# ecpoppenheimer/TensorFlowRayTrace

Measured on AMD Instinct MI355X. Metric: ray-surface intersection tests/sec (fwd+bwd), higher is better.
Workload: dtype f32 ray state, f32 filter + f64 decisions

## Files before the change

tensorflowraytrace_amd/csrc/tfrt_trace3d.hip:

```cpp
#include <vector>

#include <type_traits>
#include "tfrt_common.h"
#include "goal_finish.h"
#include "wave_schedule.h"

namespace tfrt {

constexpr int TILE = 512;
constexpr int KC = 24;

constexpr int ERR_CAPACITY = 1;


__global__ __launch_bounds__(BLOCK) void k_center(const double* __restrict__ fverts, int M,
                                                  double* __restrict__ c0, int32_t* nrays0, int n,
                                                  int32_t* tail8, unsigned int* scan_ticket) {
  if (nrays0 != nullptr) {
    if (threadIdx.x == 0) *nrays0 = n;
    if (threadIdx.x < 8) tail8[threadIdx.x] = 0;
    if (threadIdx.x == 0 && scan_ticket != nullptr) *scan_ticket = 0u;
  }
  __shared__ double red[WAVES][3];
  __shared__ double ctr[3];
// ... 2552 lines not shown
    } else {
      double* gp = g_fverts + 9 * (int64_t)tri;
#pragma unroll
      for (int c = 0; c < 9; ++c)
        if (gP[c] != 0.0) unsafeAtomicAdd(gp + c, gP[c]);
    }
  }
  wave_fence();
  for (int k0 = 0; k0 < cells; k0 += 64) {
    const int k = k0 + lane;
    double v = k < cells ? wacc[k] : 0.0;
    v += dpp_f64<0xB1>(v);
    if (copies >= 4) v += dpp_f64<0x4E>(v);
    if (copies >= 8) v += dpp_f64<0x141>(v);
    if ((lane & (copies - 1)) == 0 && k < cells && v != 0.0) {
      const int term = k / copies;
      unsafeAtomicAdd(g_fverts + 9 * (int64_t)wface[term / 9] + (term % 9), v);
    }
  }
  wave_fence();
}

template <typename T, int BW>
__global__ __launch_bounds__(64 * BW) void k_backward3d(
    const T* __restrict__ rays_in, int64_t stride_in, const int32_t* __restrict__ n_ptr,
    const int32_t* __restrict__ ray_id_in, const int32_t* __restrict__ rec_tri,
    const double* __restrict__ rec_t, const uint8_t* __restrict__ rec_cls,
    const int32_t* __restrict__ rec_slot, const int32_t* __restrict__ pass_counts,
    tfrt_scene3d sc, double L, double dead_len,
    const typename SweepStore<T>::type* __restrict__ g_child, int64_t child_stride,
    const double* __restrict__ g_fin, int64_t cap_fin, const double* __restrict__ g_act,
    int64_t cap_act, const double* __restrict__ g_stp, int64_t cap_stp,
    const double* __restrict__ g_dead, int64_t cap_dead,
    typename SweepStore<T>::type* __restrict__ g_out, double* __restrict__ g_src_out,
    int64_t out_stride, double* __restrict__ g_fverts,
    typename SweepStore<T>::type* __restrict__ stash_g, int32_t* __restrict__ stash_face,
    int wave_sums) {
  const int n = *n_ptr;
  const int q0 = blockIdx.x * (64 * BW) + threadIdx.x;
  const int i = q0;
  if (wave_sums) {
    if ((q0 & ~63) >= n) return;
    __shared__ double wacc[BW][WSUM_CELLS];
    __shared__ int32_t wface[BW][WSUM_SLOTS];
    const int wave = threadIdx.x >> 6;
    double gP[9];
    int tri = -1;
    if (i < n)
      tri = backward_ray<T>(i, rays_in, stride_in, ray_id_in, rec_tri, rec_t, rec_cls, rec_slot,
                            pass_counts, sc, L, dead_len, g_child, child_stride, g_fin, cap_fin,
                            g_act, cap_act, g_stp, cap_stp, g_dead, cap_dead, g_out, g_src_out,
                            out_stride, gP);
    wave_face_sums(tri, gP, wacc[wave], wface[wave], g_fverts);
    return;
  }
  if (i >= n) return;
  double gP[9];
  const int tri = backward_ray<T>(i, rays_in, stride_in, ray_id_in, rec_tri, rec_t, rec_cls,
                                  rec_slot, pass_counts, sc, L, dead_len, g_child, child_stride,
                                  g_fin, cap_fin, g_act, cap_act, g_stp, cap_stp, g_dead, cap_dead,
                                  g_out, g_src_out, out_stride, gP);
  if (stash_face != nullptr) {
    stash_face[i] = tri;
    if (tri >= 0) {
      using S = typename SweepStore<T>::type;
      S* o = stash_g + 9 * (int64_t)i;
#pragma unroll
      for (int c = 0; c < 9; ++c) o[c] = static_cast<S>(gP[c]);
    }
    return;
  }
  if (tri >= 0) {
    double* gp = g_fverts + 9 * (int64_t)tri;
#pragma unroll
    for (int c = 0; c < 9; ++c) {
      if (gP[c] != 0.0) unsafeAtomicAdd(gp + c, gP[c]);
    }
  }
}

constexpr int FACE_WINDOW = 2048;

template <typename S>
__global__ __launch_bounds__(1024) void k_face_accumulate(
    const int32_t* __restrict__ nrays, int passes, int64_t pass_stride,
    const int32_t* __restrict__ stash_face, const S* __restrict__ stash_g, int chunk, int M,
    double* __restrict__ g_fverts) {
  __shared__ double acc[FACE_WINDOW * 9];
  const int lo = blockIdx.x * chunk;
  if (lo >= nrays[0]) return;
  const int w0 = blockIdx.y * FACE_WINDOW;
  const int w1 = min(M, w0 + FACE_WINDOW);
  for (int k = threadIdx.x; k < FACE_WINDOW * 9; k += 1024) acc[k] = 0.0;
  __syncthreads();
  for (int p = 0; p < passes; ++p) {
    const int hi = min(nrays[p], lo + chunk);
    const int32_t* __restrict__ face = stash_face + (int64_t)p * pass_stride;
    const S* __restrict__ terms = stash_g + 9 * (int64_t)p * pass_stride;
    constexpr int U = 4;
    for (int base = lo + threadIdx.x; base < hi; base += 1024 * U) {
      int t[U];
#pragma unroll
      for (int u = 0; u < U; ++u) {
        const int i = base + u * 1024;
        t[u] = i < hi ? face[i] : -1;
      }
      double g[U][9];
#pragma unroll
      for (int u = 0; u < U; ++u) {
        if (t[u] >= w0 && t[u] < w1) {
          const S* src = terms + 9 * (int64_t)(base + u * 1024);
#pragma unroll
          for (int c = 0; c < 9; ++c) g[u][c] = static_cast<double>(src[c]);
        }
      }
#pragma unroll
      for (int u = 0; u < U; ++u) {
        if (t[u] >= w0 && t[u] < w1) {
          double* a = acc + 9 * (t[u] - w0);
#pragma unroll
          for (int c = 0; c < 9; ++c)
            if (g[u][c] != 0.0) unsafeAtomicAdd(a + c, g[u][c]);
        }
      }
    }
  }
  __syncthreads();
  for (int k = threadIdx.x; k < (w1 - w0) * 9; k += 1024) {
    const double v = acc[k];
    if (v != 0.0) unsafeAtomicAdd(g_fverts + 9 * (int64_t)w0 + k, v);
  }
}

constexpr int FIXED_BITS = 40;

template <typename S>
__global__ __launch_bounds__(BLOCK) void k_stash_absmax(const int32_t* __restrict__ n_ptr,
                                                        const int32_t* __restrict__ stash_face,
                                                        const S* __restrict__ stash_g,
                                                        unsigned long long* __restrict__ maxbits) {
  const int n = *n_ptr;
  const int i = blockIdx.x * BLOCK + threadIdx.x;
  double m = 0.0;
  if (i < n && stash_face[i] >= 0) {
    const S* g = stash_g + 9 * (int64_t)i;
#pragma unroll
    for (int c = 0; c < 9; ++c) {
      const double a = fabs(static_cast<double>(g[c]));
      if (a > m && a < INFINITY) m = a;
    }
  }
#pragma unroll
  for (int d = 32; d > 0; d >>= 1) m = fmax(m, __shfl_xor(m, d, 64));
  if (lane_id() == 0 && m > 0.0) atomicMax(maxbits, (unsigned long long)__double_as_longlong(m));
}

__device__ __forceinline__ double fixed_scale(unsigned long long maxbits) {
  if (maxbits == 0ull) return 0.0;
  int e;
  (void)frexp(__longlong_as_double((long long)maxbits), &e);
  int shift = FIXED_BITS - e;
  if (shift > 1000) shift = 1000;
  return ldexp(1.0, shift);
}

template <typename S>
__global__ __launch_bounds__(BLOCK) void k_face_accumulate_fixed(
    const int32_t* __restrict__ n_ptr, const int32_t* __restrict__ stash_face,
    const S* __restrict__ stash_g, const unsigned long long* __restrict__ maxbits,
    unsigned long long* __restrict__ acc, uint8_t* __restrict__ flag) {
  const int n = *n_ptr;
  const int i = blockIdx.x * BLOCK + threadIdx.x;
  if (i >= n) return;
  const int f = stash_face[i];
  if (f < 0) return;
  const double scale = fixed_scale(*maxbits);
  const S* g = stash_g + 9 * (int64_t)i;
#pragma unroll
  for (int c = 0; c < 9; ++c) {
    const double x = static_cast<double>(g[c]);
    if (!(fabs(x) < INFINITY)) {
      flag[9 * (int64_t)f + c] = 1;
    } else {
      const long long q = llrint(x * scale);
      if (q != 0) atomicAdd(acc + 9 * (int64_t)f + c, (unsigned long long)q);
    }
  }
}

__global__ __launch_bounds__(BLOCK) void k_fixed_finish(int64_t m9,
                                                        const unsigned long long* __restrict__ max_this,
                                                        unsigned long long* __restrict__ max_next,
                                                        unsigned long long* __restrict__ acc,
                                                        uint8_t* __restrict__ flag,
                                                        double* __restrict__ g_fverts) {
  const int64_t i = (int64_t)blockIdx.x * BLOCK + threadIdx.x;
  const double scale = fixed_scale(*max_this);
  if (i < m9) {
    const long long q = (long long)acc[i];
    if (flag[i] != 0) {
      g_fverts[i] = __builtin_nan("");
    } else if (q != 0) {
      g_fverts[i] += (double)q / scale;
    }
    acc[i] = 0ull;
    flag[i] = 0;
  }
  if (i == 0) *max_next = 0ull;
}

template <typename T, bool GN = true>
__device__ __forceinline__ int backward_core(
    int i, int tape, int slot, const T* __restrict__ rays_in, int64_t stride_in,
    const int32_t* __restrict__ ray_id_in, const int32_t* __restrict__ rec_tri,
    const double* __restrict__ rec_t, const int32_t* __restrict__ pass_counts,
    const tfrt_scene3d& sc, double L, double dead_len, bool child_pass, const double child[6],
    const double* seed_fin,
    const double* __restrict__ g_fin, int64_t cap_fin, const double* __restrict__ g_act,
    int64_t cap_act, const double* __restrict__ g_stp, int64_t cap_stp,
    const double* __restrict__ g_dead, int64_t cap_dead, double gs[3], double ge[3],
    double gP[9], int tri_known = -2, const double* __restrict__ feta = nullptr,
    bool slot_global = false) {
  int face_out = -1;
  const int cls = tape & 3;
  double s[3], e[3];
  load_ray3(rays_in, stride_in, i, s, e);
  for (int k = 0; k < 3; ++k) gs[k] = ge[k] = 0.0;
  double P[9], t_rec = 0.0, n_in = 1.0, n_out = 1.0;
  int tri = tri_known;
  auto load_face = [&](bool with_indices) {
    const double* fp = sc.face_verts + 9 * (int64_t)tri;
#pragma unroll
    for (int q = 0; q < 9; ++q) P[q] = fp[q];
    t_rec = rec_t[i];
    if (with_indices) {
      if (feta != nullptr) {
        n_in = feta[4 * (int64_t)tri + 2];
        n_out = feta[4 * (int64_t)tri + 3];
      } else {
        face_indices(sc, tri, ray_id_in ? ray_id_in[i] : i, &n_in, &n_out);
      }
    }
  };
  const bool early = tri_known >= 0 && cls != CLS_DEAD;
  if (early) load_face(child_pass && cls == CLS_ACTIVE);

  if (cls == CLS_DEAD) {
    if (g_dead != nullptr) {
      double a[3] = {0, 0, 0}, b[3] = {0, 0, 0};
      add6(g_dead, cap_dead, slot, a, b);
      const double dl = (dead_len != 0.0) ? dead_len : 1.0;
      for (int k = 0; k < 3; ++k) {
        gs[k] = a[k] + (1.0 - dl) * b[k];
        ge[k] = dl * b[k];
      }
    }
  } else {
    double g_s[3] = {0, 0, 0}, g_h[3] = {0, 0, 0}, g_ce[3] = {0, 0, 0};
    bool has_child = false;
    if (cls == CLS_FINISHED) {
      if (seed_fin != nullptr) {
        for (int k = 0; k < 3; ++k) {
          g_s[k] += seed_fin[k];
          g_h[k] += seed_fin[3 + k];
        }
      } else {
        add6(g_fin, cap_fin, slot, g_s, g_h);
      }
    } else if (cls == CLS_STOPPED) {
      add6(g_stp, cap_stp, slot, g_s, g_h);
    } else {
      if (g_act != nullptr)
        add6(g_act, cap_act, (slot_global ? 0 : (int64_t)pass_counts[4 + CLS_ACTIVE]) + slot, g_s, g_h);
      if (child_pass) {
        has_child = true;
        for (int k = 0; k < 3; ++k) {
          g_h[k] += child[k];
          g_ce[k] += child[3 + k];
        }
      }
    }
    bool nz = has_child;
    for (int k = 0; k < 3; ++k) nz = nz || g_s[k] != 0.0 || g_h[k] != 0.0;
    if (nz) {
      if (!early) {
        if (tri_known < -1) tri = rec_tri[i];
        load_face(has_child);
      }
      double gn[2];
      const bool want_n = GN && has_child && sc.grad_n_in != nullptr && sc.n_table == nullptr;
      const int branch = ((tape & TAPE_INTERNAL) ? 1 : 0) | ((tape & TAPE_REFLECT) ? 2 : 0);
      adjoint3d(s, e, P, t_rec, has_child, n_in, n_out, L, g_s, g_h, g_ce, gs, ge, gP, gn, branch,
                want_n);
      if (want_n) {
        if (gn[0] != 0.0) unsafeAtomicAdd(sc.grad_n_in + tri, gn[0]);
        if (gn[1] != 0.0) unsafeAtomicAdd(sc.grad_n_out + tri, gn[1]);
      }
      if (sc.face_grad_mask == nullptr || sc.face_grad_mask[tri] != 0) face_out = tri;
    }
  }
  return face_out;
}

template <typename T>
__device__ __forceinline__ int backward_ray(
    int i, const T* __restrict__ rays_in, int64_t stride_in, const int32_t* __restrict__ ray_id_in,
    const int32_t* __restrict__ rec_tri, const double* __restrict__ rec_t,
    const uint8_t* __restrict__ rec_cls, const int32_t* __restrict__ rec_slot,
    const int32_t* __restrict__ pass_counts, const tfrt_scene3d& sc, double L, double dead_len,
    const typename SweepStore<T>::type* __restrict__ g_child, int64_t child_stride,
    const double* __restrict__ g_fin, int64_t cap_fin, const double* __restrict__ g_act,
    int64_t cap_act, const double* __restrict__ g_stp, int64_t cap_stp,
    const double* __restrict__ g_dead, int64_t cap_dead,
    typename SweepStore<T>::type* __restrict__ g_out, double* __restrict__ g_src_out,
    int64_t out_stride, double gP[9]) {
  const int tape = rec_cls[i];
  const int slot = rec_slot[i];
  double child[6] = {0, 0, 0, 0, 0, 0};
  const bool child_pass = g_child != nullptr;
  if (child_pass && (tape & 3) == CLS_ACTIVE) {
    for (int k = 0; k < 6; ++k) child[k] = static_cast<double>(g_child[k * child_stride + slot]);
  }
  double gs[3], ge[3];
  const int face_out = backward_core<T>(i, tape, slot, rays_in, stride_in, ray_id_in, rec_tri,
                                        rec_t, pass_counts, sc, L, dead_len, child_pass, child,
                                        nullptr, g_fin, cap_fin, g_act, cap_act, g_stp, cap_stp, g_dead,
                                        cap_dead, gs, ge, gP);
  if (g_out != nullptr) {
    using G = typename SweepStore<T>::type;
    for (int k = 0; k < 3; ++k) {
      g_out[k * out_stride + i] = static_cast<G>(gs[k]);
      g_out[(3 + k) * out_stride + i] = static_cast<G>(ge[k]);
    }
  } else if (g_src_out != nullptr) {
    for (int k = 0; k < 3; ++k) {
      g_src_out[k * out_stride + i] = gs[k];
      g_src_out[(3 + k) * out_stride + i] = ge[k];
    }
  }
  return face_out;
}

constexpr int CHAIN_MAXP = 8;

template <typename T>
struct ChainArgs {
  const T* src;
  int64_t src_stride;
  const T* rays_ws;
  const int32_t* nrays;
  const int32_t* rayid;
  const int32_t* rec_tri;
  const int32_t* rec_slot;
  const double* rec_t;
  const uint8_t* rec_cls;
  const int32_t* counts;
  int64_t n;
  int32_t P;
  double L, dead_len;
  const double *g_fin, *g_act, *g_stp, *g_dead;
  int64_t cap_fin, cap_act, cap_stp, cap_dead;
  double* g_src;
  int64_t N;
  double* g_fverts;
  const T* fin_rays;
  int64_t fin_cap;
  GoalFields gf;
  const double* goal;
  int64_t goal_stride, goal_ray_stride;
  double* partial;
  int32_t* partial_cnt;
  const double* feta;
  int32_t inplace;
  int32_t chain_in_lds;
};

#ifndef TFRT_CHAIN_WAVES
#define TFRT_CHAIN_WAVES 4
#endif
template <typename T, int BW, bool GOAL, bool GN>
__global__ __launch_bounds__(64 * BW)
__attribute__((amdgpu_waves_per_eu(TFRT_CHAIN_WAVES, TFRT_CHAIN_WAVES))) void k_backward_chain(
    ChainArgs<T> a, tfrt_scene3d sc) {
#pragma clang fp contract(off)
  const int n0 = a.nrays[0];
  const int i0 = blockIdx.x * (64 * BW) + threadIdx.x;
  if ((i0 & ~63) >= n0) {
    if (GOAL && (threadIdx.x & 63) == 0) {
      a.partial[i0 >> 6] = 0.0;
      if (a.partial_cnt != nullptr) a.partial_cnt[2 * (i0 >> 6)] = a.partial_cnt[2 * (i0 >> 6) + 1] = 0;
    }
    return;
  }
  __shared__ double wacc[BW][WSUM_CELLS];
  __shared__ int32_t wface[BW][WSUM_SLOTS];
  extern __shared__ int4 chain_lds[];
  const int lane = threadIdx.x & 63, wave = threadIdx.x >> 6;
  const int P = a.P;
  int4* chain = chain_lds + (size_t)wave * P * 64;
  int last = -1;
  if (i0 < n0) {
    int j = i0;
    for (int p = 0; p < P; ++p) {
      const size_t at = (size_t)p * a.n + j;
      const int tape = a.rec_cls[at], tri = a.rec_tri[at];
      const int slot = a.inplace >= 2 ? j : a.rec_slot[at];
      if (a.chain_in_lds) chain[p * 64 + lane] = make_int4(j, tape, slot, tri);
      last = p;
      if ((tape & 3) != CLS_ACTIVE || p == P - 1) break;
      if (!a.inplace) j = slot;
    }
  }
  int top = last;
#pragma unroll
  for (int d = 32; d > 0; d >>= 1) top = max(top, __shfl_xor(top, d, 64));
  double child[6] = {0, 0, 0, 0, 0, 0};
  double err = 0.0;
  int n_fin = 0, n_entered = 0;
  for (int p = top; p >= 0; --p) {
    double gP[9];
    int tri = -1;
    bool fin_here = false;
    if (p <= last) {
      int4 rec;
      if (a.chain_in_lds) {
        rec = chain[p * 64 + lane];
      } else {
        const size_t at = (size_t)p * a.n + i0;
        rec = make_int4(i0, a.rec_cls[at], a.inplace >= 2 ? i0 : a.rec_slot[at], a.rec_tri[at]);
      }
      const int j = rec.x, tape = rec.y, slot = rec.z;
      const size_t off = (size_t)p * a.n;
      const T* rin = p == 0 ? a.src : a.rays_ws + (size_t)(p - 1) * 6 * a.n;
      const int64_t sin = p == 0 ? a.src_stride : a.n;
      const int32_t* idin = (p == 0 || a.inplace) ? nullptr : a.rayid + (size_t)(p - 1) * a.n;
      double seed[6] = {0, 0, 0, 0, 0, 0};
      if (GOAL && p == last && (tape & 3) == CLS_FINISHED) {
        fin_here = true;
        double fin_row[6] = {0, 0, 0, 0, 0, 0};
        if (a.inplace) {
          double s0[3], e0[3], h0[3];
          load_ray3(rin, sin, j, s0, e0);
          hit_point(s0, e0, a.rec_t[off + j], h0);
#pragma unroll
          for (int k = 0; k < 3; ++k) {
            fin_row[k] = s0[k];
            fin_row[3 + k] = static_cast<double>(static_cast<T>(h0[k]));
          }
        }
        for (int c = 0; c < a.gf.n; ++c) {
          const int row = a.gf.row[c];
          double out_c = 0.0;
          if (a.inplace) {
#pragma unroll
            for (int k = 0; k < 6; ++k)
              if (k == row) out_c = fin_row[k];
          } else {
            out_c = ldd(a.fin_rays, (int64_t)row * a.fin_cap + slot);
          }
          const double r = out_c -
                           a.goal[(int64_t)c * a.goal_stride + (int64_t)i0 * a.goal_ray_stride];
          const double g = 2.0 * r;
#pragma unroll
          for (int q = 0; q < 6; ++q)
            if (q == row) seed[q] = g;
          err += r * r;
        }
      }
      double gs[3], ge[3];
      tri = backward_core<T, GN>(j, tape, slot, rin, sin, idin, a.rec_tri + off, a.rec_t + off,
                                 a.counts + (size_t)p * TFRT_COUNTS_PER_PASS, sc, a.L, a.dead_len,
                                 p < P - 1, child, GOAL ? seed : nullptr, a.g_fin, a.cap_fin, a.g_act,
                             a.cap_act, a.g_stp, a.cap_stp, a.g_dead, a.cap_dead, gs, ge, gP,
                             rec.w, a.feta, a.inplace != 0);
      for (int k = 0; k < 3; ++k) {
        child[k] = gs[k];
        child[3 + k] = ge[k];
      }
    }
    if (GOAL) {
      n_fin += __popcll(__ballot(fin_here));
      n_entered += __popcll(__ballot(p <= last));
    }
    wave_face_sums(tri, gP, wacc[wave], wface[wave], a.g_fverts);
  }
  if (a.g_src != nullptr && i0 < n0) {
    for (int k = 0; k < 6; ++k) a.g_src[k * a.N + i0] = child[k];
  }
  if (GOAL) {
#pragma unroll
    for (int d = 32; d > 0; d >>= 1) err += __shfl_xor(err, d, 64);
    if (lane == 0) {
      a.partial[i0 >> 6] = err;
      if (a.partial_cnt != nullptr) {
        a.partial_cnt[2 * (i0 >> 6)] = n_fin;
        a.partial_cnt[2 * (i0 >> 6) + 1] = n_entered;
      }
    }
  }
}

template <typename T>
struct ChainGoalArgs {
  const T* src;
  int64_t src_stride;
  const T* rays_ws;
  const int32_t* nrays;
  const int32_t* rec_tri;
  const double* rec_t;
  const uint8_t* rec_cls;
  int64_t n;
  int32_t P;
  double L;
  double* g_src;
  int64_t N;
  double* g_fverts;
  GoalFields gf;
  const double* goal;
  int64_t goal_stride, goal_ray_stride;
  double* partial;
  int32_t* partial_cnt;
  const double* feta;
  const double* face_verts;
  const uint8_t* face_grad_mask;
  const int32_t* sched;
  int32_t ngroups;
};

template <typename T>
__global__ __launch_bounds__(64)
__attribute__((amdgpu_waves_per_eu(TFRT_CHAIN_WAVES, TFRT_CHAIN_WAVES))) void k_backward_chain_goal_inplace(
    ChainGoalArgs<T> a) {
#pragma clang fp contract(off)
  const int n0 = a.nrays[0];
  int wave = blockIdx.x;
  if (a.sched != nullptr) {
    wave = __builtin_amdgcn_readfirstlane(a.sched[blockIdx.x]);
    if ((unsigned)wave >= (unsigned)a.ngroups) return;
  }
  const int i0 = wave * 64 + threadIdx.x;
  const int lane = threadIdx.x;
  if ((i0 & ~63) >= n0) {
    if (lane == 0) {
      a.partial[i0 >> 6] = 0.0;
      if (a.partial_cnt != nullptr) a.partial_cnt[2 * (i0 >> 6)] = a.partial_cnt[2 * (i0 >> 6) + 1] = 0;
    }
    return;
  }
  __builtin_assume(a.feta != nullptr);
  __shared__ double wacc[WSUM_CELLS];
  __shared__ int32_t wface[WSUM_SLOTS];
  extern __shared__ int2 chain_goal_lds[];
  int2* chain = chain_goal_lds;
  const int P = a.P;
  tfrt_scene3d sc = {};
  sc.face_verts = a.face_verts;
  sc.face_grad_mask = a.face_grad_mask;
  int last = -1;
  if (i0 < n0) {
    for (int p = 0; p < P; ++p) {
      const size_t at = (size_t)p * a.n + i0;
      const int tape = a.rec_cls[at], tri = a.rec_tri[at];
      chain[p * 64 + lane] = make_int2(tape, tri);
      last = p;
      if ((tape & 3) != CLS_ACTIVE) break;
    }
  }
  int top = last;
#pragma unroll
  for (int d = 32; d > 0; d >>= 1) top = max(top, __shfl_xor(top, d, 64));
  top = __builtin_amdgcn_readfirstlane(top);
  double child[6] = {0, 0, 0, 0, 0, 0};
  double err = 0.0;
  int n_fin = 0, n_entered = 0;
  for (int p = top; p >= 0; --p) {
    double gP[9];
    int tri = -1;
    bool fin_here = false;
    if (p <= last) {
      const int2 rec = chain[p * 64 + lane];
      const int tape = rec.x;
      const size_t off = (size_t)p * a.n;
      const T* rin = p == 0 ? a.src : a.rays_ws + (size_t)(p - 1) * 6 * a.n;
      const int64_t sin = p == 0 ? a.src_stride : a.n;
      double seed[6] = {0, 0, 0, 0, 0, 0};
      if (p == last && (tape & 3) == CLS_FINISHED) {
        fin_here = true;
        double fin_row[6], s0[3], e0[3], h0[3];
        load_ray3(rin, sin, i0, s0, e0);
        hit_point(s0, e0, a.rec_t[off + i0], h0);
#pragma unroll
        for (int k = 0; k < 3; ++k) {
          fin_row[k] = s0[k];
          fin_row[3 + k] = static_cast<double>(static_cast<T>(h0[k]));
        }
        for (int c = 0; c < a.gf.n; ++c) {
          const int row = a.gf.row[c];
          double out_c = 0.0;
#pragma unroll
          for (int k = 0; k < 6; ++k)
            if (k == row) out_c = fin_row[k];
          const double r = out_c -
                           a.goal[(int64_t)c * a.goal_stride + (int64_t)i0 * a.goal_ray_stride];
          const double g = 2.0 * r;
#pragma unroll
          for (int q = 0; q < 6; ++q)
            if (q == row) seed[q] = g;
          err += r * r;
        }
      }
      double gs[3], ge[3];
      tri = backward_core<T, false>(i0, tape, i0, rin, sin, nullptr, a.rec_tri + off, a.rec_t + off,
                                    nullptr, sc, a.L, 0.0, p < P - 1, child, seed, nullptr, 0,
                                    nullptr, 0, nullptr, 0, nullptr, 0, gs, ge, gP,
                                    max(rec.y, -1),
                                    a.feta, true);
      for (int k = 0; k < 3; ++k) {
        child[k] = gs[k];
        child[3 + k] = ge[k];
      }
    }
    n_fin += __popcll(__ballot(fin_here));
    n_entered += __popcll(__ballot(p <= last));
    wave_face_sums(tri, gP, wacc, wface, a.g_fverts);
  }
  if (a.g_src != nullptr && i0 < n0) {
    for (int k = 0; k < 6; ++k) a.g_src[k * a.N + i0] = child[k];
  }
#pragma unroll
  for (int d = 32; d > 0; d >>= 1) err += __shfl_xor(err, d, 64);
  if (lane == 0) {
    a.partial[i0 >> 6] = err;
    if (a.partial_cnt != nullptr) {
      a.partial_cnt[2 * (i0 >> 6)] = n_fin;
      a.partial_cnt[2 * (i0 >> 6) + 1] = n_entered;
    }
  }
}


template <typename T>
__global__ __launch_bounds__(BLOCK) void k_finalize_seam(
    const T* __restrict__ rays, int64_t stride, int n, int chunks,
    const double* __restrict__ part_t, const int32_t* __restrict__ part_i, int64_t part_stride,
    const double* __restrict__ fverts, int M, double eps_int, double eps_size, double eps_start,
    double* x, double* y, double* z, uint8_t* valid, double* ray_u, double* trig_u,
    double* trig_v, int32_t* gather_trig) {
  const int i = blockIdx.x * BLOCK + threadIdx.x;
  if (i >= n) return;
  double bt = INFINITY;
  int bi = -1;
  for (int c = 0; c < chunks; ++c) {
    const double t = part_t[c * part_stride + i];
    if (t < bt) {
      bt = t;
      bi = part_i[c * part_stride + i];
    }
  }
  const int tri = bi < 0 ? 0 : bi;
  double s[3], e[3], P[9], h[3] = {0, 0, 0};
  TriHit th;
  th.ray_u = th.trig_u = th.trig_v = 0.0;
  th.valid = false;
  if (M > 0) {
    load_ray3(rays, stride, i, s, e);
    for (int q = 0; q < 9; ++q) P[q] = fverts[9 * (int64_t)tri + q];
    th = exact_triangle(s, e, P, eps_int, eps_size, eps_start);
    hit_point(s, e, th.ray_u, h);
  }
  x[i] = h[0];
  y[i] = h[1];
  z[i] = h[2];
  valid[i] = bi >= 0;
  ray_u[i] = bi >= 0 ? th.ray_u : INFINITY;
  trig_u[i] = th.trig_u;
  trig_v[i] = th.trig_v;
  gather_trig[i] = tri;
}


struct Plan3 {
  int R, ray_blocks, chunks, chunk_faces, nblk;
  int g_blocks, g_chunks, g_chunk_clusters;
};

struct Accel3 {
  const int32_t* order;
  int n_clusters;
  float4* csphere;
  int32_t* cface;
  float4* clsphere;
  float4* susphere;
  float4* crec;
};

static Plan3 make_plan(int64_t N, int64_t M) {
  Plan3 p;
  p.R = (N >= 32768) ? 4 : (N >= 8192 ? 2 : 1);
  p.ray_blocks = cdiv(N > 0 ? N : 1, (int64_t)BLOCK * p.R);
  int target = 4096;
  int chunks = cdiv(target, p.ray_blocks);
  const int max_chunks = cdiv(M > 0 ? M : 1, 256);
  if (chunks > max_chunks) chunks = max_chunks;
  if (chunks < 1) chunks = 1;
  p.chunk_faces = cdiv(M > 0 ? M : 1, chunks);
  p.chunks = cdiv(M > 0 ? M : 1, p.chunk_faces);
  p.nblk = cdiv(N > 0 ? N : 1, BLOCK);
  const int n_clusters = cdiv(M > 0 ? M : 1, 16);
  p.g_blocks = cdiv(N > 0 ? N : 1, (int64_t)BLOCK);
  int gtarget = 64;
  int gch = cdiv(gtarget, p.g_blocks);
  const int gmax = cdiv(n_clusters, 64);
  if (gch > gmax) gch = gmax;
  if (gch > p.chunks) gch = p.chunks;
  if (gch < 1) gch = 1;
  p.g_chunk_clusters = (cdiv(n_clusters, gch) + 7) / 8 * 8;
  p.g_chunks = cdiv(n_clusters, p.g_chunk_clusters);
  return p;
}

struct Layout3 {
  size_t c0, sphere, nrays, blockcnt, blockoff, rowtot, rowbase, ticket, part_t, part_i, prep;
  size_t csphere, cface, clsphere, susphere, crec, fnorm, feta, hist_a, hist_b, left_list, wcount,
      wbase, tape_args;
  size_t rays, rayid, lasttri, rec_tri, rec_slot, rec_t, rec_cls, gbuf, stash_g, stash_face, fix_acc,
      fix_flag, fix_max, total;
};

static Layout3 make_layout(int64_t N, int64_t M, int P, int dtype, const Plan3& pl) {
  Layout3 L;
  const size_t esz = state_bytes(dtype);
  const size_t n = N > 0 ? N : 1, m = M > 0 ? M : 1;
  size_t o = 0;
  auto take = [&](size_t bytes) {
    size_t at = o;
    o = align_up(o + bytes);
    return at;
  };
  L.c0 = take(4 * sizeof(double));
  L.sphere = take(m * sizeof(float4));
  L.nrays = take((P + 2) * sizeof(int32_t));
  L.blockcnt = take((size_t)pl.nblk * 4 * sizeof(int32_t));
  L.blockoff = take((size_t)pl.nblk * 4 * sizeof(int32_t));
  L.rowtot = take((size_t)cdiv(pl.nblk, 1024) * 4 * sizeof(int32_t));
  L.rowbase = take((size_t)cdiv(pl.nblk, 1024) * 4 * sizeof(int32_t));
  L.ticket = take(sizeof(unsigned int));
  L.part_t = take((size_t)pl.chunks * n * sizeof(double));
  L.part_i = take((size_t)pl.chunks * n * sizeof(int32_t));
  L.prep = take((size_t)8 * n * sizeof(float));
  const size_t ncl = (m + CLUSTER - 1) / CLUSTER;
  L.csphere = take(ncl * CLUSTER * sizeof(float4));
  L.cface = take(ncl * CLUSTER * sizeof(int32_t));
  L.clsphere = take(ncl * sizeof(float4));
  L.susphere = take((ncl + SUPER - 1) / SUPER * sizeof(float4));
  L.crec = take(ncl * CLUSTER * 3 * sizeof(float4));
  L.fnorm = take(m * 3 * sizeof(double));
  L.feta = take(m * 4 * sizeof(double));
  L.hist_a = take(((size_t)pl.nblk * 4 + 1) * sizeof(int32_t));
  L.hist_b = take(((size_t)pl.nblk * 4 + 1) * sizeof(int32_t));
  L.left_list = take((n + 63) / 64 * sizeof(int32_t));
  L.wcount = take((size_t)(2 * (P > 0 ? P : 1) + 2) * inplace_wstride(n) * sizeof(uint32_t));
  L.wbase = take((size_t)(P > 0 ? P : 1) * inplace_wstride(n) * sizeof(int4));
  L.tape_args = take(sizeof(InplaceTape));
  L.rays = take((size_t)P * 6 * n * esz);
  L.rayid = take((size_t)P * n * sizeof(int32_t));
  L.lasttri = take((size_t)P * n * sizeof(int32_t));
  L.rec_tri = take((size_t)P * n * sizeof(int32_t));
  L.rec_slot = take((size_t)P * n * sizeof(int32_t));
  L.rec_t = take((size_t)P * n * sizeof(double));
  L.rec_cls = take((size_t)P * n);
  L.gbuf = take((size_t)2 * 6 * n * sizeof(double));
  L.stash_g = take((size_t)(P > 0 ? P : 1) * 9 * n * sizeof(double));
  L.stash_face = take((size_t)(P > 0 ? P : 1) * n * sizeof(int32_t));
  L.fix_acc = take((size_t)9 * m * sizeof(unsigned long long));
  L.fix_flag = take((size_t)9 * m);
  L.fix_max = take(2 * sizeof(unsigned long long));
  L.total = o;
  return L;
}

template <typename T>
struct Tape3 {
  template <typename U>
  using as = std::conditional_t<std::is_const_v<T>, const U, U>;
  using E = std::remove_const_t<T>;
  as<char>* ws;
  const Layout3& lay;
  size_t n;
  template <typename U>
  as<U>* at(size_t offset) const { return reinterpret_cast<as<U>*>(ws + offset); }
  Tape3(as<void>* workspace, const Layout3& layout, int64_t N)
      : ws(static_cast<as<char>*>(workspace)), lay(layout), n(N > 0 ? N : 1) {}

  as<int32_t>* nrays = at<int32_t>(lay.nrays);
  as<double>* fnorm = at<double>(lay.fnorm);
  as<double>* feta = at<double>(lay.feta);
  as<uint32_t>* wcount = at<uint32_t>(lay.wcount);
  as<int4>* wbase = at<int4>(lay.wbase);
  as<InplaceTape>* tape_args = at<InplaceTape>(lay.tape_args);
  T* rays_out(int p) const { return at<E>(lay.rays) + (size_t)p * 6 * n; }
  as<int32_t>* ids(int p) const { return at<int32_t>(lay.rayid) + (size_t)p * n; }
  as<int32_t>* last(int p) const { return at<int32_t>(lay.lasttri) + (size_t)p * n; }
  as<int32_t>* rec_tri(int p) const { return at<int32_t>(lay.rec_tri) + (size_t)p * n; }
  as<int32_t>* rec_slot(int p) const { return at<int32_t>(lay.rec_slot) + (size_t)p * n; }
  as<double>* rec_t(int p) const { return at<double>(lay.rec_t) + (size_t)p * n; }
  as<uint8_t>* rec_cls(int p) const { return at<uint8_t>(lay.rec_cls) + (size_t)p * n; }
  PassIn<E> input(int p, const void* src, int64_t src_stride) const {
    if (p == 0) return {static_cast<const E*>(src), src_stride, nullptr, nullptr};
    return {rays_out(p - 1), (int64_t)n, ids(p - 1), last(p - 1)};
  }
};

struct ProfRec {
  hipEvent_t a, b;
  int32_t kind;
};
static bool g_prof_on = false;
static std::vector<ProfRec> g_prof;
struct ProfScope {
  ProfRec rec;
  hipStream_t st;
  bool on;
  ProfScope(int kind, hipStream_t stream) : st(stream), on(g_prof_on) {
    if (!on) return;
    rec.kind = kind;
    (void)hipEventCreate(&rec.a);
    (void)hipEventCreate(&rec.b);
    (void)hipEventRecord(rec.a, st);
  }
  ~ProfScope() {
    if (!on) return;
    (void)hipEventRecord(rec.b, st);
    g_prof.push_back(rec);
  }
};

struct Classify3 {
  const int32_t* catagory = nullptr;
  int32_t* rec_tri = nullptr;
  double* rec_t = nullptr;
  uint8_t* rec_cls = nullptr;
  int32_t* blockcnt = nullptr;
};

struct Ordered3 {
  int nq = 0;
  int32_t* hist = nullptr;
  int32_t* left_list = nullptr;
  int32_t* left_count = nullptr;
  int32_t* left_total = nullptr;
  int coherent_only = 0;
  int n_super = 0;
};

template <typename T>
static int launch_intersect(const Plan3& pl, hipStream_t st, const T* rays, int64_t stride,
                            const int32_t* n_ptr, const int32_t* last_tri, const float4* sphere,
                            const double* fverts, const double* c0, float* prep, int64_t pstride,
                            int M, double ei, double es, double er, double* part_t,
                            int32_t* part_i, int64_t part_stride, const Accel3* ac,
                            bool prep_ready = false, const Classify3* classify = nullptr,
                            bool* classified = nullptr, const Ordered3* od = nullptr) {
  const bool grouped = ac != nullptr && ac->order != nullptr;
  Classify3 fz;
  if (grouped && pl.g_chunks == 1 && classify != nullptr && classify->rec_cls != nullptr)
    fz = *classify;
  if (classified != nullptr) *classified = fz.rec_cls != nullptr;
  const bool prep_inline = grouped && !prep_ready;
  if (!prep_ready && !prep_inline)
    hipLaunchKernelGGL((k_rayprep<T>), dim3(pl.nblk), dim3(BLOCK), 0, st, rays, stride, n_ptr, c0,
                       prep, pstride);
  dim3 grid(pl.ray_blocks, pl.chunks);
  if (grouped) grid = dim3(pl.g_blocks, pl.g_chunks);
  ProfScope prof(TFRT_PROF_INTERSECT, st);
  if (grouped && od != nullptr) {
    int bundle = 64;
    if (od->coherent_only && od->nq <= 160 * 1024) bundle = 32;
    constexpr int BEAM_BW = 1;
    const BeamScene bs = {ac->susphere, ac->clsphere, ac->csphere, ac->crec, fverts, c0,
                          ac->n_clusters, od->n_super, ei, es, er};
    hipLaunchKernelGGL((k_intersect_beam<T, BEAM_BW>), dim3(cdiv(od->nq, BEAM_BW * bundle)),
                       dim3(64 * BEAM_BW), 0, st, rays, stride, n_ptr, last_tri, bs, fz.catagory,
                       fz.rec_tri, fz.rec_t, fz.rec_cls, od->hist, od->left_list,
                       od->left_count, od->left_total, od->coherent_only, bundle);
    grid = dim3(min(cdiv(od->nq, BLOCK), 1280), 1);
  }
  if (grouped && od != nullptr) {
    if (!od->coherent_only)
      hipLaunchKernelGGL((k_intersect_group_left<T>), grid, dim3(BLOCK), 0, st, rays, stride, n_ptr,
                         last_tri, ac->susphere, ac->clsphere, ac->csphere, ac->crec, ac->cface,
                         fverts, c0, ac->n_clusters, pl.g_chunk_clusters, ei, es, er, fz.catagory,
                         fz.rec_tri, fz.rec_t, fz.rec_cls, od->left_list, od->left_count, od->hist);
  } else if (grouped) {
    hipLaunchKernelGGL((k_intersect_group<T>), grid, dim3(BLOCK), 0, st, rays, stride, n_ptr,
                       last_tri, ac->susphere, ac->clsphere, ac->csphere, ac->crec, ac->cface,
                       fverts, c0, prep_inline ? nullptr : prep, pstride, ac->n_clusters,
                       pl.g_chunk_clusters, ei, es, er, part_t, part_i, part_stride, fz.catagory,
                       fz.rec_tri, fz.rec_t, fz.rec_cls, fz.blockcnt);
  } else {
#define TFRT_LAUNCH_R(RR)                                                                      \
    hipLaunchKernelGGL((k_intersect3d<T, RR>), grid, dim3(BLOCK), 0, st, rays, stride, n_ptr,  \
                       last_tri, sphere, fverts, prep, pstride, M, pl.chunk_faces, ei, es, er, \
                       part_t, part_i, part_stride)
    if (pl.R == 1) { TFRT_LAUNCH_R(1); }
    else if (pl.R == 4) { TFRT_LAUNCH_R(4); }
    else { TFRT_LAUNCH_R(2); }
#undef TFRT_LAUNCH_R
  }
  return 0;
}

static bool scene_ok(const tfrt_scene3d* sc) {
  if (!sc || sc->n_faces < 0) return false;
  if (sc->n_faces > 0 && (!sc->face_verts || !sc->catagory)) return false;
  if (sc->n_faces >= (1ll << 29)) return false;
  const bool index_mode = sc->mat_in && sc->mat_out && sc->n_table;
  const bool value_mode = sc->n_in && sc->n_out;
  return sc->n_faces == 0 || index_mode || value_mode;
}
// ... 759 lines not shown
```

tensorflowraytrace_amd/csrc/trace_math.h:

```cpp
#pragma once
#include <math.h>

#if defined(__HIPCC__)
#define TFRT_HD __host__ __device__ __forceinline__
#else
#define TFRT_HD inline
#endif

namespace tfrt {

constexpr int CLS_ACTIVE = 0;
constexpr int CLS_FINISHED = 1;
constexpr int CLS_STOPPED = 2;
constexpr int CLS_DEAD = 3;

constexpr int CAT_OPTICAL = 0, CAT_STOP = 1, CAT_TARGET = 2;

struct TriHit {
  double ray_u, trig_u, trig_v;
  bool valid;
};

TFRT_HD TriHit exact_triangle(const double s[3], const double e[3], const double P[9],
                              double eps_int, double eps_size, double eps_start) {
#pragma clang fp contract(off)
  const double a = s[0] - e[0], d = s[1] - e[1], h = s[2] - e[2];
  const double b = P[3] - P[0], f = P[4] - P[1], k = P[5] - P[2];
  const double c = P[6] - P[0], g = P[7] - P[1], l = P[8] - P[2];
  const double q = s[0] - P[0], r = s[1] - P[1], t = s[2] - P[2];

  const double den = a * g * k + b * d * l + c * f * h - a * f * l - b * g * h - c * d * k;
  const double nr = b * l * r + c * f * t + g * k * q - b * g * t - c * k * r - f * l * q;
  const double nu = a * g * t + c * h * r + d * l * q - a * l * r - c * d * t - g * h * q;
  const double nv = a * k * r + b * d * t + f * h * q - a * f * t - b * h * r - d * k * q;

  TriHit o;
  bool valid = fabs(den) >= eps_int;
  const double sd = valid ? den : 1.0;
  o.ray_u = nr / sd;
  o.trig_u = nu / sd;
  o.trig_v = nv / sd;
  valid = valid && (o.trig_u >= -eps_size);
  valid = valid && (o.trig_v >= -eps_size);
  valid = valid && (o.trig_u + o.trig_v <= 1.0 + eps_size);
  valid = valid && (o.ray_u >= eps_start);
  o.valid = valid;
  return o;
}

TFRT_HD void hit_point(const double s[3], const double e[3], double ray_u, double h[3]) {
#pragma clang fp contract(off)
  h[0] = s[0] - ray_u * (s[0] - e[0]);
  h[1] = s[1] - ray_u * (s[1] - e[1]);
  h[2] = s[2] - ray_u * (s[2] - e[2]);
}

TFRT_HD double advance(double origin, double L, double dir) {
#pragma clang fp contract(off)
  return origin + L * dir;
}

TFRT_HD double advance_between(double s, double L, double e) {
#pragma clang fp contract(off)
  return s + L * (e - s);
}

TFRT_HD void cross3(const double a[3], const double b[3], double o[3]) {
#pragma clang fp contract(off)
  o[0] = a[1] * b[2] - a[2] * b[1];
  o[1] = a[2] * b[0] - a[0] * b[2];
  o[2] = a[0] * b[1] - a[1] * b[0];
}

TFRT_HD double dot3(const double a[3], const double b[3]) {
#pragma clang fp contract(off)
  return a[0] * b[0] + a[1] * b[1] + a[2] * b[2];
}

TFRT_HD void face_normal(const double P[9], double N[3], double C[3], double* clen) {
#pragma clang fp contract(off)
  const double A[3] = {P[3] - P[0], P[4] - P[1], P[5] - P[2]};
  const double B[3] = {P[6] - P[3], P[7] - P[4], P[8] - P[5]};
  cross3(A, B, C);
  const double len = sqrt(dot3(C, C));
  *clen = len;
  N[0] = C[0] / len;
  N[1] = C[1] / len;
  N[2] = C[2] / len;
}

TFRT_HD double l2_normalize3(const double v[3], double o[3]) {
#pragma clang fp contract(off)
  double sq = dot3(v, v);
  if (sq < 1e-12) sq = 1e-12;
  const double inv = 1.0 / sqrt(sq);
  o[0] = v[0] * inv;
  o[1] = v[1] * inv;
  o[2] = v[2] * inv;
  return inv;
}

struct Snell3 {
  double u[3], n[3];
  double nu, eta, k;
  bool reflect;
  double w[3];
};

TFRT_HD void snell_normal(const double P[9], double n[3]) {
  double N[3], C[3], clen;
  face_normal(P, N, C, &clen);
  l2_normalize3(N, n);
}

TFRT_HD void snell_ratios(double n_in, double n_out, double* n1, double* n2) {
#pragma clang fp contract(off)
  const bool in_safe = n_in != 0.0, out_safe = n_out != 0.0;
  const double nis = in_safe ? n_in : 1.0, nos = out_safe ? n_out : 1.0;
  *n1 = out_safe ? nis / nos : 0.0;
  *n2 = in_safe ? nos / nis : 0.0;
}

TFRT_HD Snell3 snell3d_core(const double s[3], const double h[3], const double un[3], double n1,
                            double n2, bool mirror) {
#pragma clang fp contract(off)
  Snell3 o;
  const double r[3] = {h[0] - s[0], h[1] - s[1], h[2] - s[2]};
  l2_normalize3(r, o.u);
  o.n[0] = un[0];
  o.n[1] = un[1];
  o.n[2] = un[2];
  o.nu = dot3(o.n, o.u);
  const bool internal = o.nu > 0.0;
  o.eta = internal ? n1 : n2;
  const double nu_eta = o.eta * o.nu;
  o.k = 1.0 - o.eta * o.eta + nu_eta * nu_eta;
  const bool tir = o.k < 0.0;
  o.reflect = tir || mirror;
  if (o.reflect) {
    for (int i = 0; i < 3; ++i) o.w[i] = -2.0 * o.nu * o.n[i] + o.u[i];
  } else {
    const double sg = (o.nu > 0.0) ? 1.0 : ((o.nu < 0.0) ? -1.0 : 0.0);
    const double alpha = sg * sqrt(o.k) - nu_eta;
    for (int i = 0; i < 3; ++i) o.w[i] = alpha * o.n[i] + o.eta * o.u[i];
  }
  return o;
}

TFRT_HD Snell3 snell3d_unit(const double s[3], const double h[3], const double un[3],
                            double n_in, double n_out) {
  double n1, n2;
  snell_ratios(n_in, n_out, &n1, &n2);
  return snell3d_core(s, h, un, n1, n2, n_in == 0.0);
}

TFRT_HD Snell3 snell3d(const double s[3], const double h[3], const double norm[3],
                       double n_in, double n_out) {
  double un[3];
  l2_normalize3(norm, un);
  return snell3d_unit(s, h, un, n_in, n_out);
}

TFRT_HD double fmod_floor(double x, double m) {
  double r = fmod(x, m);
  if (r != 0.0 && ((r < 0.0) != (m < 0.0))) r += m;
  return r;
}

TFRT_HD double snell2d_angle(double xs, double ys, double xe, double ye, double norm,
                             double n_in, double n_out) {
#pragma clang fp contract(off)
  const double PI = 3.141592653589793;
  norm = fmod_floor(norm, 2 * PI);
  double ray_angle = atan2(ys - ye, xs - xe);
  ray_angle = fmod_floor(ray_angle, 2 * PI);
  double theta1 = norm - ray_angle;
  if (theta1 > PI) theta1 = theta1 - 2 * PI;
  if (theta1 < -PI) theta1 = theta1 + 2 * PI;
  const bool internal = fabs(theta1) >= PI / 2;
  const bool in_safe = n_in != 0.0, out_safe = n_out != 0.0;
  const double nis = in_safe ? n_in : 1.0, nos = out_safe ? n_out : 1.0;
  const double n1 = out_safe ? nis / nos : 0.0;
  const double n2 = in_safe ? nos / nis : 0.0;
  const double n = internal ? n1 : n2;
  if (!internal) norm = norm + PI;
  if (internal) theta1 = theta1 + PI;
  const double theta2 = n * sin(theta1);
  if (fabs(theta2) <= 1.0 && n != 0.0) return norm - asin(theta2);
  return norm + theta1 + PI;
}

TFRT_HD double adj_rcp(double x) {
#if defined(__HIP_DEVICE_COMPILE__)
  double r = __builtin_amdgcn_rcp(x);
  r = __builtin_fma(__builtin_fma(-x, r, 1.0), r, r);
  r = __builtin_fma(__builtin_fma(-x, r, 1.0), r, r);
  return r;
#else
  return 1.0 / x;
#endif
}
TFRT_HD double adj_rsqrt(double x) {
#if defined(__HIP_DEVICE_COMPILE__)
  double y = __builtin_amdgcn_rsq(x);
  double e = __builtin_fma(-x * y, y, 1.0);
  y = __builtin_fma(0.5 * y, e, y);
  e = __builtin_fma(-x * y, y, 1.0);
  y = __builtin_fma(0.5 * y, e, y);
  return y;
#else
  return 1.0 / sqrt(x);
#endif
}

TFRT_HD void adjoint3d(const double s[3], const double e[3], const double P[9], double ray_u,
                       bool has_child, double n_in, double n_out, double L,
                       const double g_s[3], const double g_h[3], const double g_ce[3],
                       double gs[3], double ge[3], double gP[9], double* gn = nullptr,
                       int branch = -1, bool gn_wanted = true) {
  if (gn != nullptr) gn[0] = gn[1] = 0.0;
  const double d[3] = {e[0] - s[0], e[1] - s[1], e[2] - s[2]};
  const double E1[3] = {P[3] - P[0], P[4] - P[1], P[5] - P[2]};
  const double E2[3] = {P[6] - P[0], P[7] - P[1], P[8] - P[2]};
  double C[3];
  cross3(E1, E2, C);
  const double t = ray_u;
  double h[3] = {s[0] + t * d[0], s[1] + t * d[1], s[2] + t * d[2]};

  double hb[3] = {g_h[0], g_h[1], g_h[2]};
  double sb[3] = {g_s[0], g_s[1], g_s[2]};
  for (int i = 0; i < 9; ++i) gP[i] = 0.0;

  if (has_child) {
    const double inv_c = adj_rsqrt(dot3(C, C));
    const double n[3] = {C[0] * inv_c, C[1] * inv_c, C[2] * inv_c};
    const double r[3] = {h[0] - s[0], h[1] - s[1], h[2] - s[2]};
    const double rsq = dot3(r, r);
    const bool clamped = rsq < 1e-12;
    const double inv_r = clamped ? 1e6 : adj_rsqrt(rsq);
    const double u[3] = {r[0] * inv_r, r[1] * inv_r, r[2] * inv_r};
    const double nu = dot3(n, u);
    const bool in_safe = n_in != 0.0, out_safe = n_out != 0.0;
    const double nis = in_safe ? n_in : 1.0, nos = out_safe ? n_out : 1.0;
    const bool internal = branch >= 0 ? (branch & 1) != 0 : nu > 0.0;
    const double eta = internal ? (out_safe ? nis / nos : 0.0) : (in_safe ? nos / nis : 0.0);
    const double nu_eta = eta * nu;
    double k = 1.0 - eta * eta + nu_eta * nu_eta;
    const bool reflect = branch >= 0 ? (branch & 2) != 0 : ((k < 0.0) || (n_in == 0.0));
    if (!reflect && k < 0.0) k = 0.0;
    double wb[3], ub[3], nb[3];
    for (int i = 0; i < 3; ++i) {
      hb[i] += g_ce[i];
      wb[i] = L * g_ce[i];
    }
    double nub;
    if (reflect) {
      nub = -2.0 * dot3(wb, n);
      for (int i = 0; i < 3; ++i) {
        ub[i] = wb[i];
        nb[i] = -2.0 * nu * wb[i];
      }
    } else {
      const double sg = branch >= 0 ? (internal ? 1.0 : (nu < 0.0 ? -1.0 : 0.0))
                                    : ((nu > 0.0) ? 1.0 : ((nu < 0.0) ? -1.0 : 0.0));
      const double irk = k > 0.0 ? adj_rsqrt(k) : INFINITY;
      const double rk = k > 0.0 ? k * irk : 0.0;
      const double alpha = sg * rk - nu_eta;
      const double ab = dot3(wb, n);
      nub = ab * (sg * eta * nu_eta * irk - eta);
      if (gn != nullptr && gn_wanted) {
        const double etab = dot3(wb, u) + ab * (sg * eta * (nu * nu - 1.0) * irk - nu);
        if (internal) {
          if (out_safe) {
            gn[0] = in_safe ? etab / nos : 0.0;
            gn[1] = -etab * eta / nos;
          }
        } else if (in_safe) {
          gn[1] = out_safe ? etab / nis : 0.0;
          gn[0] = -etab * eta / nis;
        }
      }
      for (int i = 0; i < 3; ++i) {
        nb[i] = alpha * wb[i];
        ub[i] = eta * wb[i];
      }
    }
    for (int i = 0; i < 3; ++i) {
      nb[i] += nub * u[i];
      ub[i] += nub * n[i];
    }
    if (!clamped) {
      const double uu = dot3(u, ub);
      for (int i = 0; i < 3; ++i) {
        const double rb = (ub[i] - u[i] * uu) * inv_r;
        hb[i] += rb;
        sb[i] -= rb;
      }
    } else {
      for (int i = 0; i < 3; ++i) {
        hb[i] += ub[i] * 1e6;
        sb[i] -= ub[i] * 1e6;
      }
    }
    const double nn = dot3(n, nb);
    double Cb[3];
    for (int i = 0; i < 3; ++i) Cb[i] = (nb[i] - n[i] * nn) * inv_c;
    double E1b[3], E2b[3];
    cross3(E2, Cb, E1b);
    cross3(Cb, E1, E2b);
    for (int i = 0; i < 3; ++i) {
      gP[3 + i] += E1b[i];
      gP[6 + i] += E2b[i];
      gP[i] -= E1b[i] + E2b[i];
    }
  }

  double db[3];
  double tb = 0.0;
  for (int i = 0; i < 3; ++i) {
    sb[i] += hb[i];
    tb += hb[i] * d[i];
    db[i] = t * hb[i];
  }
  const double den = dot3(d, C);
  const double numb = tb * adj_rcp(den);
  const double denb = -numb * t;
  double Cb[3];
  for (int i = 0; i < 3; ++i) {
    gP[i] += numb * C[i];
    sb[i] -= numb * C[i];
    Cb[i] = numb * (P[i] - s[i]) + denb * d[i];
    db[i] += denb * C[i];
  }
  double E1b[3], E2b[3];
  cross3(E2, Cb, E1b);
  cross3(Cb, E1, E2b);
  for (int i = 0; i < 3; ++i) {
    gP[3 + i] += E1b[i];
    gP[6 + i] += E2b[i];
    gP[i] -= E1b[i] + E2b[i];
    ge[i] = db[i];
    gs[i] = sb[i] - db[i];
  }
}

}
```

Before: 123900 billion.

## Prefetch per-pass backward loads up front and merge adjoint cross-product terms

In the fused goal/backward wave kernel, each pass now issues all of its global loads together before any arithmetic: ray state, recorded t, goal values, face vertices, the grad mask and refractive indices. It then calls a new backward_core_loaded that works only on registers, instead of the generic backward_core that loaded its inputs inside. The aim is to overlap load latency and cut dependent waits per pass, at the cost of extra live registers and some loads done speculatively. Separately, adjoint3d folds the normal-derivative C gradient into the intersection C gradient, so only one pair of cross products runs and gP is written once rather than zeroed and accumulated. A scratch script for counting instructions in the assembly is also added.

Result: faster. 126500 billion, median of 6 (+2.1%).

```diff
diff --git a/scratch/kcount.py b/scratch/kcount.py
--- /dev/null
+++ b/scratch/kcount.py
@@ -0,0 +1,76 @@
+#!/usr/bin/env python3
+import argparse, re, subprocess
+
+ap = argparse.ArgumentParser()
+ap.add_argument("asm"); ap.add_argument("res"); ap.add_argument("filt", nargs="?", default="")
+ap.add_argument("--loads", default=None)
+a = ap.parse_args()
+asm, res, filt, loads = a.asm, a.res, a.filt, a.loads
+
+remarks, cur = {}, None
+for line in open(res):
+    m = re.search(r"remark: +(.*?) \[-Rpass", line)
+    if not m:
+        continue
+    t = m.group(1).strip()
+    if t.startswith("Function Name:"):
+        cur = remarks.setdefault(t.split(":", 1)[1].strip(), {})
+    elif cur is not None and ":" in t:
+        k, v = t.split(":", 1)
+        cur[k.strip()] = v.strip()
+
+kernels, name = {}, None
+for line in open(asm):
+    m = re.match(r"^(_Z\w+):", line)
+    if m and m.group(1) in remarks:
+        name = m.group(1)
+        kernels[name] = []
+        continue
+    if name is not None:
+        t = line.strip()
+        if t and not t.startswith((";", ".")) or re.match(r"^\.LBB", t):
+            kernels[name].append(t)
+        if t.startswith("s_endpgm"):
+            name = None
+
+names = list(kernels)
+dem = subprocess.run(["c++filt"] + names, stdout=subprocess.PIPE).stdout.decode().splitlines()
+F64 = re.compile(r"^v_(add|mul|fma|div\w*|rcp|rsq|sqrt)_f64")
+print(f"{'kernel':52s} {'SGPR':>4s} {'VGPR':>4s} {'sspill':>6s} {'vsp':>3s} {'scr':>4s} {'occ':>3s} {'LDS':>6s} {'v_':>5s} {'s_':>5s} {'lane':>4s} {'f64':>4s} {'*_f64':>5s}")
+for n, d in zip(names, dem):
+    d = re.sub(r"\(.*", "", d).replace("void tfrt::", "").replace("tfrt::", "")
+    if filt and filt not in d:
+        continue
+    ins = [t.split()[0] for t in kernels[n] if not t.endswith(":") and not t.startswith(".LBB")]
+    r = remarks[n]
+    v = sum(i.startswith("v_") for i in ins)
+    s = sum(i.startswith("s_") for i in ins)
+    lane = sum(i.startswith(("v_readlane", "v_writelane")) for i in ins)
+    f64 = sum(bool(F64.match(i)) for i in ins)
+    any64 = sum(bool(re.search(r"_f64(_e32|_e64)?$", i)) for i in ins)
+    print(f"{d[:52]:52s} {r.get('TotalSGPRs', '?'):>4s} {r.get('VGPRs', '?'):>4s} {r.get('SGPRs Spill', '?'):>6s} "
+          f"{r.get('VGPRs Spill', '?'):>3s} {r.get('ScratchSize [bytes/lane]', '?'):>4s} {r.get('Occupancy [waves/SIMD]', '?'):>3s} "
+          f"{r.get('LDS Size [bytes/block]', '?'):>6s} {v:5d} {s:5d} {lane:4d} {f64:4d} {any64:5d}")
+
+if loads:
+    for n, d in zip(names, dem):
+        if loads not in d:
+            continue
+        body = kernels[n]
+        heads = [i for i, t in enumerate(body) if re.match(r"^\.LBB\d+_\d+:.*Loop Header: Depth=1", t)]
+        for h in heads:
+            label = body[h].split(":")[0]
+            tag = label[1:]
+            tag = tag[1:] if tag.startswith("L") else tag
+            seg, inside = [], False
+            for t in body[h:]:
+                if re.match(r"^\.LBB\d+_\d+:", t):
+                    inside = t.startswith(label + ":") or ("Header=" + tag) in t or ("Parent Loop " + tag) in t
+                elif inside:
+                    seg.append(t)
+            if sum("global_load" in t for t in seg) >= 6:
+                print(f"\n{d[:70]}: global loads and waits for them in the pass loop ({label}), in layout order")
+                for t in seg:
+                    if t.startswith("global_load") or (t.startswith("s_waitcnt") and "vmcnt" in t):
+                        print("   ", t.split(";")[0].strip())
+                break
diff --git a/tensorflowraytrace_amd/csrc/tfrt_trace3d.hip b/tensorflowraytrace_amd/csrc/tfrt_trace3d.hip
--- a/tensorflowraytrace_amd/csrc/tfrt_trace3d.hip
+++ b/tensorflowraytrace_amd/csrc/tfrt_trace3d.hip
@@ -2878,6 +2878,40 @@
   return face_out;
 }
 
+__device__ __forceinline__ int backward_core_loaded(
+    int tape, int tri, bool child_pass, const double s[3], const double e[3], const double P[9],
+    double t_rec, double n_in, double n_out, bool face_wanted, double L, const double child[6],
+    const double seed[6], double gs[3], double ge[3], double gP[9]) {
+  int face_out = -1;
+  const int cls = tape & 3;
+  for (int k = 0; k < 3; ++k) gs[k] = ge[k] = 0.0;
+  if (cls != CLS_DEAD) {
+    double g_s[3] = {0, 0, 0}, g_h[3] = {0, 0, 0}, g_ce[3] = {0, 0, 0};
+    bool has_child = false;
+    if (cls == CLS_FINISHED) {
+      for (int k = 0; k < 3; ++k) {
+        g_s[k] += seed[k];
+        g_h[k] += seed[3 + k];
+      }
+    } else if (cls == CLS_ACTIVE && child_pass) {
+      has_child = true;
+      for (int k = 0; k < 3; ++k) {
+        g_h[k] += child[k];
+        g_ce[k] += child[3 + k];
+      }
+    }
+    bool nz = has_child;
+    for (int k = 0; k < 3; ++k) nz = nz || g_s[k] != 0.0 || g_h[k] != 0.0;
+    if (nz) {
+      const int branch = ((tape & TAPE_INTERNAL) ? 1 : 0) | ((tape & TAPE_REFLECT) ? 2 : 0);
+      adjoint3d(s, e, P, t_rec, has_child, n_in, n_out, L, g_s, g_h, g_ce, gs, ge, gP, nullptr,
+                branch, false);
+      if (face_wanted) face_out = tri;
+    }
+  }
+  return face_out;
+}
+
 template <typename T>
 __device__ __forceinline__ int backward_ray(
     int i, const T* __restrict__ rays_in, int64_t stride_in, const int32_t* __restrict__ ray_id_in,
@@ -3129,9 +3163,6 @@
   extern __shared__ int2 chain_goal_lds[];
   int2* chain = chain_goal_lds;
   const int P = a.P;
-  tfrt_scene3d sc = {};
-  sc.face_verts = a.face_verts;
-  sc.face_grad_mask = a.face_grad_mask;
   int last = -1;
   if (i0 < n0) {
     for (int p = 0; p < P; ++p) {
@@ -3155,29 +3186,69 @@
     bool fin_here = false;
     if (p <= last) {
       const int2 rec = chain[p * 64 + lane];
-      const int tape = rec.x;
+      const int tape = rec.x, cls = tape & 3;
+      const int face = max(rec.y, -1);
       const size_t off = (size_t)p * a.n;
       const T* rin = p == 0 ? a.src : a.rays_ws + (size_t)(p - 1) * 6 * a.n;
       const int64_t sin = p == 0 ? a.src_stride : a.n;
+      const bool child_pass = p < P - 1;
+      fin_here = p == last && cls == CLS_FINISHED;
+      const bool on_face = face >= 0 && cls != CLS_DEAD;
+      const bool with_child = on_face && child_pass && cls == CLS_ACTIVE;
+      int iv = i0;
+      __asm__ volatile("" : "+v"(iv));
+      T ray_w[6];
+#pragma unroll
+      for (int k = 0; k < 6; ++k) ray_w[k] = rin[k * sin + iv];
+      double t_rec = 0.0;
+      if (fin_here || on_face) t_rec = a.rec_t[off + iv];
+      double goal_w[6];
+#pragma unroll
+      for (int c = 0; c < 6; ++c) {
+        goal_w[c] = 0.0;
+        if (fin_here && c < a.gf.n)
+          goal_w[c] = a.goal[(int64_t)c * a.goal_stride + (int64_t)iv * a.goal_ray_stride];
+      }
+      double Pf[9] = {0, 0, 0, 0, 0, 0, 0, 0, 0}, n_in = 1.0, n_out = 1.0;
+      uint8_t mask_w = 1;
+      if (on_face) {
+        const double* fp = a.face_verts + 9 * (int64_t)face;
+#pragma unroll
+        for (int q = 0; q < 9; ++q) Pf[q] = fp[q];
+        if (a.face_grad_mask != nullptr && (with_child || cls == CLS_FINISHED))
+          mask_w = a.face_grad_mask[face];
+      }
+      if (with_child) {
+        n_in = a.feta[4 * (int64_t)face + 2];
+        n_out = a.feta[4 * (int64_t)face + 3];
+      }
+      double s0[3], e0[3];
+#pragma unroll
+      for (int k = 0; k < 3; ++k) {
+        s0[k] = static_cast<double>(ray_w[k]);
+        e0[k] = static_cast<double>(ray_w[3 + k]);
+      }
+      int mask_i = mask_w;
+      __asm__ volatile("" : "+v"(mask_i));
       double seed[6] = {0, 0, 0, 0, 0, 0};
-      if (p == last && (tape & 3) == CLS_FINISHED) {
-        fin_here = true;
-        double fin_row[6], s0[3], e0[3], h0[3];
-        load_ray3(rin, sin, i0, s0, e0);
-        hit_point(s0, e0, a.rec_t[off + i0], h0);
+      if (fin_here) {
+        double fin_row[6], h0[3];
+        hit_point(s0, e0, t_rec, h0);
 #pragma unroll
         for (int k = 0; k < 3; ++k) {
           fin_row[k] = s0[k];
           fin_row[3 + k] = static_cast<double>(static_cast<T>(h0[k]));
         }
+#pragma nounroll
         for (int c = 0; c < a.gf.n; ++c) {
           const int row = a.gf.row[c];
-          double out_c = 0.0;
-#pragma unroll
-          for (int k = 0; k < 6; ++k)
+          double out_c = 0.0, goal_c = 0.0;
+#pragma unroll
+          for (int k = 0; k < 6; ++k) {
             if (k == row) out_c = fin_row[k];
-          const double r = out_c -
-                           a.goal[(int64_t)c * a.goal_stride + (int64_t)i0 * a.goal_ray_stride];
+            if (k == c) goal_c = goal_w[k];
+          }
+          const double r = out_c - goal_c;
           const double g = 2.0 * r;
 #pragma unroll
           for (int q = 0; q < 6; ++q)
@@ -3186,11 +3257,8 @@
         }
       }
       double gs[3], ge[3];
-      tri = backward_core<T, false>(i0, tape, i0, rin, sin, nullptr, a.rec_tri + off, a.rec_t + off,
-                                    nullptr, sc, a.L, 0.0, p < P - 1, child, seed, nullptr, 0,
-                                    nullptr, 0, nullptr, 0, nullptr, 0, gs, ge, gP,
-                                    max(rec.y, -1),
-                                    a.feta, true);
+      tri = backward_core_loaded(tape, face, child_pass, s0, e0, Pf, t_rec, n_in, n_out,
+                                 mask_i != 0, a.L, child, seed, gs, ge, gP);
       for (int k = 0; k < 3; ++k) {
         child[k] = gs[k];
         child[3 + k] = ge[k];
diff --git a/tensorflowraytrace_amd/csrc/trace_math.h b/tensorflowraytrace_amd/csrc/trace_math.h
--- a/tensorflowraytrace_amd/csrc/trace_math.h
+++ b/tensorflowraytrace_amd/csrc/trace_math.h
@@ -229,7 +229,7 @@
 
   double hb[3] = {g_h[0], g_h[1], g_h[2]};
   double sb[3] = {g_s[0], g_s[1], g_s[2]};
-  for (int i = 0; i < 9; ++i) gP[i] = 0.0;
+  double Cn[3] = {0.0, 0.0, 0.0};
 
   if (has_child) {
     const double inv_c = adj_rsqrt(dot3(C, C));
@@ -303,16 +303,7 @@
       }
     }
     const double nn = dot3(n, nb);
-    double Cb[3];
-    for (int i = 0; i < 3; ++i) Cb[i] = (nb[i] - n[i] * nn) * inv_c;
-    double E1b[3], E2b[3];
-    cross3(E2, Cb, E1b);
-    cross3(Cb, E1, E2b);
-    for (int i = 0; i < 3; ++i) {
-      gP[3 + i] += E1b[i];
-      gP[6 + i] += E2b[i];
-      gP[i] -= E1b[i] + E2b[i];
-    }
+    for (int i = 0; i < 3; ++i) Cn[i] = (nb[i] - n[i] * nn) * inv_c;
   }
 
   double db[3];
@@ -327,18 +318,17 @@
   const double denb = -numb * t;
   double Cb[3];
   for (int i = 0; i < 3; ++i) {
-    gP[i] += numb * C[i];
     sb[i] -= numb * C[i];
-    Cb[i] = numb * (P[i] - s[i]) + denb * d[i];
+    Cb[i] = Cn[i] + (numb * (P[i] - s[i]) + denb * d[i]);
     db[i] += denb * C[i];
   }
   double E1b[3], E2b[3];
   cross3(E2, Cb, E1b);
   cross3(Cb, E1, E2b);
   for (int i = 0; i < 3; ++i) {
-    gP[3 + i] += E1b[i];
-    gP[6 + i] += E2b[i];
-    gP[i] -= E1b[i] + E2b[i];
+    gP[3 + i] = E1b[i];
+    gP[6 + i] = E2b[i];
+    gP[i] = numb * C[i] - (E1b[i] + E2b[i]);
     ge[i] = db[i];
     gs[i] = sb[i] - db[i];
   }
```
